# qiqiqicheng/news-recommendation-tc

Measured on AMD Instinct MI355X. Metric: recalled pairs/sec (YouTubeDNN top-30) + DIN scored pairs/sec, 1/2/4/8 MI355X, higher is better.
Workload: dtype fp16

## Files before the change

news-recommendation-tc_amd/csrc/ip_topk.hip:

```cpp
#include "nrk_common.h"

#include <float.h>
#include <math.h>
#include <stdlib.h>

#include <algorithm>
#include <type_traits>
#include <utility>

namespace nrk {

typedef float f32x16 __attribute__((ext_vector_type(16)));
typedef _Float16 f16x8 __attribute__((ext_vector_type(8)));
typedef unsigned u32x4 __attribute__((ext_vector_type(4)));
typedef float f32x4 __attribute__((ext_vector_type(4)));

constexpr int IP_KFAST = 128;
constexpr int IP_KMAX = 2048;
#ifndef NRK_SCAN_TILE
#define NRK_SCAN_TILE 8192
#endif
constexpr int SCAN_TILE = NRK_SCAN_TILE;
#ifndef NRK_SCAN_TB128
#define NRK_SCAN_TB128 4
#endif
__host__ __device__ constexpr int scan_tb(int dp) {
    return dp == 128 ? NRK_SCAN_TB128 : (64 * dp >= SCAN_TILE ? 1 : SCAN_TILE / (64 * dp));
}
constexpr int IP_SEL = 512;
constexpr int IP_BQ = 288;
constexpr int IP_KRING = 256;
constexpr size_t CATALOG_HDR = 256;

__host__ __device__ static inline int pad_dim(int d) {
    return d <= 16 ? 16 : d <= 32 ? 32 : d <= 64 ? 64 : d <= 128 ? 128 : 256;
}
__host__ __device__ static inline int64_t n_blocks_of(int64_t n_items) { return (n_items + 31) / 32; }

struct CatalogHdr {
    float max_norm;
    float max_abs;
    float scale;
    int32_t dim;
    int32_t dp;
    float max_dnorm;
};

__device__ __forceinline__ float pow2_scale(float maxabs) {
    if (!(maxabs > 0.0f)) return 1.0f;
    int e;
    (void)frexpf(maxabs, &e);
    return ldexpf(1.0f, 14 - e);
}

static inline size_t catalog_body_bytes(int64_t n_items, int dp) {
    return (size_t)n_blocks_of(n_items) * 64u * (size_t)dp;
}
__host__ __device__ static inline bool catalog_has_hb(int dp) { return dp <= 64; }
__host__ __device__ static inline size_t catalog_hb_offset(int64_t n_items, int dp) {
// ... 1185 lines not shown
        if (user < n_users) {
            acnt[(size_t)user * 2 + h] = (int)cnt[g];
            if (h == 0) reinterpret_cast<float*>(uinfo + user)[0] = live[g] ? lb : -INFINITY;
        }
    }
    if constexpr (MT <= 32) {
        if (bnd != nullptr) {
#pragma unroll
            for (int g = 0; g < UGB; ++g)
                list_bound_out<MT>(t[g], live[g], h, ubase + (gb + g) * 32 + q, n_users, jk, bnd, bnd_m, uinfo);
        }
    }
}

__device__ __forceinline__ uint32_t fkey(float f) {
    const uint32_t b = __float_as_uint(f);
    return (b >> 31) ? ~b : (b | 0x80000000u);
}
__device__ __forceinline__ float fkey_inv(uint32_t k) {
    return __uint_as_float((k >> 31) ? (k & 0x7FFFFFFFu) : ~k);
}

template <int E>
__device__ __forceinline__ void lds_ranks(const uint32_t* __restrict__ row, int c, const uint32_t (&mine)[E],
                                          int pos, int (&rank)[E]) {
#pragma unroll
    for (int e = 0; e < E; ++e) rank[e] = 0;
    for (int j0 = 0; j0 < c; j0 += 4) {
        const uint4 q = *reinterpret_cast<const uint4*>(row + j0);
        const uint32_t qq[4] = {q.x, q.y, q.z, q.w};
#pragma unroll
        for (int t = 0; t < 4; ++t) {
#pragma unroll
            for (int e = 0; e < E; ++e)
                rank[e] += (qq[t] > mine[e] || (qq[t] == mine[e] && j0 + t < e * WAVE + pos)) ? 1 : 0;
        }
    }
}

__device__ __forceinline__ uint32_t wave_sort_desc_u32(uint32_t x, int lane) {
    static_for<6>([&](auto klc) {
        constexpr int kl = decltype(klc)::value + 1, k = 1 << kl;
        static_for<kl>([&](auto jc) {
            constexpr int j = 1 << (kl - 1 - decltype(jc)::value);
            const uint32_t y = lane_xor<j>(x);
            const bool up = (lane & k) == 0;
            const bool lower = (lane & j) == 0;
            x = (lower == up) ? max(x, y) : min(x, y);
        });
    });
    return x;
}

__device__ __forceinline__ uint32_t lds_select(uint32_t* __restrict__ row, int c, int r, int lane) {
    if (c <= WAVE) {
        wave_sync_lds();
        const uint32_t srt = wave_sort_desc_u32(lane < c ? row[lane] : 0u, lane);
        return (uint32_t)__builtin_amdgcn_readlane((int)srt, r);
    }
    if (lane < 4) row[c + lane] = 0u;
    wave_sync_lds();
    uint32_t x = 0u;
    for (int b0 = 0; b0 < c; b0 += WAVE) {
        const uint32_t mine[1] = {b0 + lane < c ? row[b0 + lane] : 0u};
        int rank[1];
        lds_ranks<1>(row, c, mine, b0 + lane, rank);
        const unsigned long long b = __ballot(b0 + lane < c && rank[0] == r);
        if (b) {
            x = (uint32_t)__shfl((int)mine[0], __ffsll((long long)b) - 1, WAVE);
            break;
        }
    }
    return x;
}

#ifndef NRK_SH_WG
#define NRK_SH_WG 6
#endif
constexpr int SH_WG_PER_CU = NRK_SH_WG;
constexpr int SH_ENT = 4;

__device__ __forceinline__ void sh_load(const uint2* s0, const uint2* s1, int a0, int n, int b0, int lane,
                                        uint2 (&ent)[SH_ENT]) {
#pragma unroll
    for (int j = 0; j < SH_ENT; ++j) {
        const int e = b0 + j * WAVE + lane;
        ent[j] = e < n ? (e < a0 ? s0[e] : s1[e - a0]) : make_uint2(0u, 0u);
    }
}

__global__ __launch_bounds__(256) void ip_select_kernel(
    int64_t n_users, int k, int m2, int bandcap, const uint2* __restrict__ app,
    const int32_t* __restrict__ acnt, const float4* __restrict__ uinfo, uint2* __restrict__ cand,
    int32_t* __restrict__ cand_cnt, float2* __restrict__ ucut, int32_t* __restrict__ ovf_flag,
    int32_t* __restrict__ ovf_list, int32_t* __restrict__ ovf_count) {
    __shared__ __attribute__((aligned(16))) uint32_t sel[4][IP_SEL + 4];
    const int lane = threadIdx.x & 63, wave = threadIdx.x >> 6;
    const int64_t nw = (int64_t)gridDim.x * 4;
    const unsigned long long lt = (1ull << lane) - 1ull;
    int64_t u = (int64_t)blockIdx.x * 4 + wave;
    int2 ac_n = make_int2(0, 0);
    float4 inf_n = make_float4(0.f, 0.f, 0.f, 0.f);
    if (u < n_users) {
        ac_n = reinterpret_cast<const int2*>(acnt)[u];
        inf_n = uinfo[u];
    }
// ... 71 lines not shown
    for (int64_t u = blockIdx.x * (int64_t)blockDim.x + threadIdx.x; u < n_users;
         u += (int64_t)gridDim.x * blockDim.x) {
        cand_cnt[u] = 0;
        ovf_flag[u] = 1;
        ovf_list[u] = (int32_t)u;
    }
    if (blockIdx.x == 0 && threadIdx.x == 0) *ovf_count = (int32_t)n_users;
}

__device__ __forceinline__ double exact_dot(const float* __restrict__ a, const float* __restrict__ b,
                                            int dim) {
    double s = 0.0;
    if ((dim & 31) == 0) {
        const float4* a4 = reinterpret_cast<const float4*>(a);
        const float4* b4 = reinterpret_cast<const float4*>(b);
        for (int t0 = 0; t0 < dim / 4; t0 += 8) {
            float4 x[8], y[8];
#pragma unroll
            for (int t = 0; t < 8; ++t) {
                x[t] = a4[t0 + t];
                y[t] = b4[t0 + t];
            }
#pragma unroll
            for (int t = 0; t < 8; ++t) {
                s += (double)x[t].x * (double)y[t].x;
                s += (double)x[t].y * (double)y[t].y;
                s += (double)x[t].z * (double)y[t].z;
                s += (double)x[t].w * (double)y[t].w;
            }
        }
    } else if ((dim & 3) == 0) {
        const float4* a4 = reinterpret_cast<const float4*>(a);
        const float4* b4 = reinterpret_cast<const float4*>(b);
        for (int t = 0; t < dim / 4; ++t) {
            const float4 x = a4[t], y = b4[t];
            s += (double)x.x * (double)y.x;
            s += (double)x.y * (double)y.y;
            s += (double)x.z * (double)y.z;
            s += (double)x.w * (double)y.w;
        }
    } else {
        for (int t = 0; t < dim; ++t) s += (double)a[t] * (double)b[t];
    }
    return s + 0.0;
}

#ifndef NRK_REFINE_DIRECT
#define NRK_REFINE_DIRECT 1
#endif
constexpr bool REFINE_DIRECT = NRK_REFINE_DIRECT;
#ifndef NRK_REFINE_WPE
#define NRK_REFINE_WPE 6
#endif
template <int DS4, int SV>
__global__ __launch_bounds__(256) __attribute__((amdgpu_waves_per_eu(DS4 == 16 ? 2 : DS4 == 0 ? 4 : NRK_REFINE_WPE))) void ip_refine_kernel(
    const float* __restrict__ users, int64_t n_users, const float* __restrict__ items,
    const uint8_t* __restrict__ catalog, int64_t n_items, int dim, int k, int64_t row_offset,
    const uint2* __restrict__ cand, int bandcap, const int32_t* __restrict__ cand_cnt,
    const float2* __restrict__ ucut, const int32_t* __restrict__ ovf_flag, int32_t* __restrict__ ovf_list,
    int32_t* __restrict__ ovf_count, float* __restrict__ out_s, int32_t* __restrict__ out_r,
    double* __restrict__ out_e, int n_src = 0,
    int64_t src_users = 0, int x_cap = 0, const int32_t* __restrict__ src_cnt = nullptr) {
    constexpr int SE = SV / WAVE;
    __shared__ Cand surv[4][SV];
    __shared__ int32_t krow[4][IP_KRING];
    constexpr int RS = DS4 + 1;
    __shared__ float4 stage[DS4 > 0 ? 4 : 1][DS4 > 0 ? 32 * RS : 1];
    __shared__ uint32_t bandq[4][SV + 32 > IP_BQ ? SV + 32 : IP_BQ];
    __shared__ __attribute__((aligned(16))) float ushl[4][DS4 > 0 ? 1 : 256];
    const int lane = threadIdx.x & 63, wave = threadIdx.x >> 6;
    const int64_t u = (int64_t)blockIdx.x * 4 + wave;
    if (u >= n_users) return;
    const bool slots = n_src == 0;
    const float* uv = users + u * dim;
    const int32_t ovf_u = ovf_flag[u];
    const int nbd_slots = slots ? cand_cnt[u] : 0;
    const float2 ce = ucut[u];
    const float uv_r = uv[lane < dim ? lane : 0];
    const uint2 ent0 = slots ? cand[(size_t)u * bandcap + (lane < 32 ? lane : 0)] : make_uint2(0u, 0u);
    if (ovf_u) return;
    int src_n = 0;
    int nsrc_tot = 0;
    if (n_src > 0) {
        for (int s0 = 0; s0 < n_src; s0 += WAVE) {
            const int sl = s0 + lane;
            const int c = sl < n_src ? max(0, src_cnt[(int64_t)sl * src_users + u]) : 0;
            if (s0 == 0) src_n = c;
            nsrc_tot += (int)wave_sum_f32((float)c);
        }
    }
    if (nsrc_tot > IP_BQ) {
        if ((threadIdx.x & 63) == 0) ovf_list[atomicAdd(ovf_count, 1)] = (int32_t)u;
        return;
    }
    const float uv_l = lane < dim ? uv_r : 0.0f;
    float nz = fabsf(uv_l), uam = fabsf(uv_l);
    for (int d = lane + WAVE; d < dim; d += WAVE) {
        nz += fabsf(uv[d]);
        uam = fmaxf(uam, fabsf(uv[d]));
    }
    nz = wave_sum_f32(nz);
    if (nz == 0.0f) {
        for (int i = lane; i < k; i += WAVE) {
            const bool ok = i < n_items;
            out_s[u * k + i] = ok ? 0.0f : -FLT_MAX;
            out_r[u * k + i] = ok ? (int32_t)(i + row_offset) : -1;
            if (out_e) out_e[u * k + i] = ok ? 0.0 : -INFINITY;
// ... 19 lines not shown
        float ua = uam;
#pragma unroll
        for (int m = 32; m > 0; m >>= 1) ua = fmaxf(ua, __shfl_xor(ua, m, WAVE));
        const float su = pow2_scale(ua);
        if constexpr (DS4 > 0) {
#pragma unroll
            for (int d = lane; d < 4 * DS4; d += WAVE) ush[d] = (_Float16)(uv[d] * su);
            wave_sync_lds();
        }
        pcut = ce.x * (su * hdr->scale);
    }
    int nband = 0;
    auto take_one = [&](uint2 ent, int e, int cnt) {
        const bool kp = e < cnt && (!pre || __uint_as_float(ent.x) >= pcut);
        const unsigned long long bal = __ballot(kp);
        if (kp) bandq[wave][nband + __popcll(bal & ((1ull << lane) - 1ull))] = ent.y;
        nband += __popcll(bal);
    };
    auto take = [&](const uint2* __restrict__ src, int cnt) {
        int b0 = 0;
        if (slots) {
            take_one(ent0, lane < 32 ? lane : cnt, cnt);
            b0 = 32;
        }
        for (; b0 < cnt; b0 += WAVE) {
            const int e = b0 + lane;
            take_one(e < cnt ? src[e] : make_uint2(0u, 0u), e, cnt);
        }
    };
    if (n_src > 0) {
        const uint32_t* ids = reinterpret_cast<const uint32_t*>(cand);
        for (int s2 = 0; s2 < n_src; ++s2) {
            const int c2 = s2 < WAVE ? __shfl(src_n, s2, WAVE) : max(0, src_cnt[(int64_t)s2 * src_users + u]);
            const uint32_t* src = ids + ((size_t)s2 * src_users + u) * x_cap;
            for (int b0 = 0; b0 < c2; b0 += WAVE) {
                const int e = b0 + lane;
                if (e < c2) bandq[wave][nband + e] = src[e];
                nband += min(WAVE, c2 - b0);
            }
        }
    } else {
        take(bd, nbd);
    }
    wave_sync_lds();
    const int nitem = nband * 16;
    int cnt = 0;
    auto push = [&](bool keep, double s, int32_t row) {
        const unsigned long long bal = __ballot(keep);
        const int pos = cnt + __popcll(bal & ((1ull << lane) - 1ull));
        if (keep && pos < SV) surv[wave][pos] = Cand{s, row};
        cnt += __popcll(bal);
    };
    if constexpr (DS4 > 0) {
        uint4 pc[DSK > 0 ? 2 * DSK : 1];
        auto band_q = [&](int base) -> uint32_t {
            int idx = base + lane;
            idx = idx < nitem ? idx : nitem - 1;
            return bandq[wave][idx > 0 ? idx >> 4 : 0];
        };
        const uint8_t* hbc = catalog ? catalog + catalog_hb_offset(n_items, 4 * DS4) : nullptr;
        int64_t hoff = 0;
        auto item_row = [&](int base, uint32_t qv, int32_t& row, bool& inb) {
            const int idx = base + lane, r = idx & 15;
            const int64_t rr = (int64_t)(qv >> 1) * 32 + (r & 3) + 8 * (r >> 2) + 4 * (qv & 1);
            inb = idx < nitem && rr < n_items;
            row = inb ? (int32_t)rr : 0;
            hoff = inb ? ((int64_t)qv * 16 + r) * (8 * DS4) : 0;
        };
        auto pieces = [&](int32_t) {
            if (pre) {
                const uint8_t* bp = hbc + hoff;
#pragma unroll
                for (int st = 0; st < DSK; ++st)
#pragma unroll
                    for (int hh = 0; hh < 2; ++hh)
                        pc[2 * st + hh] = *reinterpret_cast<const uint4*>(bp + 32 * st + 16 * hh);
            }
        };
        int kc = 0, ko = 0;
        auto exact_round = [&](int m) {
            const int32_t rl = lane < m ? krow[wave][(ko + lane) & (IP_KRING - 1)] : -1;
            double sd = 0.0;
            bool keep = false;
            if constexpr (REFINE_DIRECT && DS4 <= 8) {
                if (rl >= 0) {
                    const float4* a4 = reinterpret_cast<const float4*>(uv);
                    const float4* b4 = reinterpret_cast<const float4*>(items + (int64_t)rl * dim);
                    constexpr int YH = DS4 > 4 ? DS4 / 2 : DS4;
                    double acc = 0.0;
#pragma unroll
                    for (int t0 = 0; t0 < DS4; t0 += YH) {
                        float4 y[YH];
#pragma unroll
                        for (int t = 0; t < YH; ++t) y[t] = b4[t0 + t];
#pragma unroll
                        for (int t = 0; t < YH; ++t) {
                            const float4 x = a4[t0 + t];
                            acc += (double)x.x * (double)y[t].x;
                            acc += (double)x.y * (double)y[t].y;
                            acc += (double)x.z * (double)y[t].z;
                            acc += (double)x.w * (double)y[t].w;
                        }
                    }
                    sd = acc + 0.0;
                    keep = sd >= thr;
                }
                push(keep, sd, rl);
                ko += m;
                return;
            }
#pragma unroll
            for (int hp = 0; hp < 2; ++hp) {
                float4 v[DS4 / 2];
                bool okv[DS4 / 2];
#pragma unroll
                for (int it = 0; it < DS4 / 2; ++it) {
                    const int g = it * 64 + lane, item = 32 * hp + g / DS4, part = g % DS4;
                    const int r_item = __shfl(rl, item, WAVE);
                    okv[it] = r_item >= 0;
                    v[it] = reinterpret_cast<const float4*>(items + (int64_t)(okv[it] ? r_item : 0) * dim)[part];
                }
#pragma unroll
                for (int it = 0; it < DS4 / 2; ++it) {
                    const int g = it * 64 + lane, part = g % DS4;
                    stage[wave][(g / DS4) * RS + part] = okv[it] ? v[it] : make_float4(0.f, 0.f, 0.f, 0.f);
                }
                wave_sync_lds();
                if ((lane >> 5) == hp && rl >= 0) {
                    const float4* a4 = reinterpret_cast<const float4*>(uv);
                    const float4* b4 = &stage[wave][(lane & 31) * RS];
                    double acc = 0.0;
#pragma unroll
                    for (int t = 0; t < DS4; ++t) {
                        const float4 x = a4[t], y = b4[t];
                        acc += (double)x.x * (double)y.x;
                        acc += (double)x.y * (double)y.y;
                        acc += (double)x.z * (double)y.z;
                        acc += (double)x.w * (double)y.w;
                    }
                    sd = acc + 0.0;
                    keep = sd >= thr;
                }
                wave_sync_lds();
            }
            push(keep, sd, rl);
            ko += m;
        };
        int32_t row;
        bool inb;
        item_row(0, band_q(0), row, inb);
        pieces(row);
        uint32_t q1 = band_q(WAVE < nitem ? WAVE : 0);
        for (int base = 0; base < nitem; base += WAVE) {
            bool keep = inb;
            if (pre && inb) {
                float acc = 0.0f;
#pragma unroll
                for (int st = 0; st < DSK; ++st)
#pragma unroll
                    for (int hh = 0; hh < 2; ++hh) {
                        const f16x8 hv = __builtin_bit_cast(f16x8, pc[2 * st + hh]);
                        const f16x8 uh = *reinterpret_cast<const f16x8*>(&ush[16 * st + 8 * hh]);
#pragma unroll
                        for (int e = 0; e < 8; ++e)
                            acc = fmaf((float)hv[e], (float)uh[e], acc);
                    }
                keep = acc >= pcut;
            }
            const int32_t row_cur = row;
            const int nb = base + WAVE;
            if (nb < nitem) {
                item_row(nb, q1, row, inb);
                pieces(row);
                q1 = band_q(nb + WAVE < nitem ? nb + WAVE : nb);
            }
            const unsigned long long bal = __ballot(keep);
            if (keep) krow[wave][(kc + __popcll(bal & ((1ull << lane) - 1ull))) & (IP_KRING - 1)] = row_cur;
            kc += __popcll(bal);
            wave_sync_lds();
            while (kc - ko >= WAVE) exact_round(WAVE);
        }
        while (kc > ko) exact_round(kc - ko < WAVE ? kc - ko : WAVE);
    } else {
        const int dpc = pad_dim(dim), dskc = dpc / 16;
        if (pre) {
            float ua = 0.0f;
            for (int d = 0; d < dim; ++d) ua = fmaxf(ua, fabsf(uv[d]));
            const float s2 = pow2_scale(ua);
            for (int d = lane; d < dpc; d += WAVE) ushl[wave][d] = d < dim ? (float)(_Float16)(uv[d] * s2) : 0.0f;
            wave_sync_lds();
        }
        int kc = 0, ko = 0;
        auto exact_generic = [&](int m) {
            const int32_t rl = lane < m ? krow[wave][(ko + lane) & (IP_KRING - 1)] : -1;
            double sd = 0.0;
            bool keep = false;
            if (rl >= 0) {
                sd = exact_dot(uv, items + (int64_t)rl * dim, dim);
                keep = sd >= thr;
            }
            push(keep, sd, rl);
            ko += m;
        };
        for (int base = 0; base < nitem; base += WAVE) {
            const int idx = base + lane;
            bool keep = false;
            int32_t row = 0;
            if (idx < nitem) {
                const int bb = idx >> 4, r = idx & 15;
                const uint32_t qv = bandq[wave][bb];
                const int64_t rr = (int64_t)(qv >> 1) * 32 + (r & 3) + 8 * (r >> 2) + 4 * (qv & 1);
                if (rr < n_items) row = (int32_t)rr;
                keep = rr < n_items;
                if (keep && pre) {
                    const uint8_t* bp = catalog + (size_t)(rr >> 5) * (64 * dpc);
                    const int il = (int)(rr & 31);
                    float acc = 0.0f;
                    for (int st = 0; st < dskc; ++st) {
                        const f16x8 h0 = __builtin_bit_cast(f16x8, *reinterpret_cast<const uint4*>(bp + st * 1024 + il * 16));
                        const f16x8 h1 =
                            __builtin_bit_cast(f16x8, *reinterpret_cast<const uint4*>(bp + st * 1024 + (il + 32) * 16));
                        const float* us = &ushl[wave][16 * st];
#pragma unroll
                        for (int e = 0; e < 8; ++e) acc = fmaf((float)h0[e], us[e], acc);
#pragma unroll
                        for (int e = 0; e < 8; ++e) acc = fmaf((float)h1[e], us[8 + e], acc);
                    }
                    keep = acc >= pcut;
                }
            }
            const unsigned long long bal = __ballot(keep);
            if (keep) krow[wave][(kc + __popcll(bal & ((1ull << lane) - 1ull))) & (IP_KRING - 1)] = row;
            kc += __popcll(bal);
            wave_sync_lds();
            while (kc - ko >= WAVE) exact_generic(WAVE);
        }
        while (kc > ko) exact_generic(kc - ko < WAVE ? kc - ko : WAVE);
    }
    if (cnt > SV) {
        if (lane == 0) ovf_list[atomicAdd(ovf_count, 1)] = (int32_t)u;
        return;
    }
    wave_sync_lds();
    auto emit = [&](const Cand* x, int ne) {
        for (int e = 0; e < ne; ++e) {
            const int idx = e * 64 + lane;
            if (idx < k) {
                const bool ok = x[e].row != INT32_MAX;
                out_s[u * k + idx] = ok ? (float)x[e].s : -FLT_MAX;
                out_r[u * k + idx] = ok ? (int32_t)(x[e].row + row_offset) : -1;
                if (out_e) out_e[u * k + idx] = ok ? x[e].s : -INFINITY;
            }
        }
    };
    if (SE > 1 && cnt <= WAVE && k <= WAVE) {
        Cand x1[1];
        if (lane < cnt) x1[0] = surv[wave][lane];
        else { x1[0].s = -INFINITY; x1[0].row = INT32_MAX; }
        wave_bitonic_sort<1>(x1);
        emit(x1, 1);
        return;
    }
    Cand x[SE];
#pragma unroll
    for (int e = 0; e < SE; ++e) {
        const int idx = e * 64 + lane;
        if (idx < cnt) x[e] = surv[wave][idx];
        else { x[e].s = -INFINITY; x[e].row = INT32_MAX; }
    }
    wave_bitonic_sort<SE>(x);
    emit(x, SE);
}

__device__ __forceinline__ uint64_t okey(double s) {
    const uint64_t b = (uint64_t)__double_as_longlong(s);
    return (b >> 63) ? ~b : (b | 0x8000000000000000ull);
}

constexpr int FB_GRID = 256;

__global__ __launch_bounds__(256) void ip_exact_kernel(
    const float* __restrict__ users, const float* __restrict__ items, int64_t n_items, int dim, int k, int ns,
    int64_t row_offset, const int32_t* __restrict__ ovf_list, const int32_t* __restrict__ ovf_count,
    float* __restrict__ out_s, int32_t* __restrict__ out_r, double* __restrict__ out_e,
    uint32_t* __restrict__ scratch, int32_t* __restrict__ slow_list, int32_t* __restrict__ slow_count) {
    extern __shared__ __attribute__((aligned(16))) uint8_t dyn[];
    Cand* sel = reinterpret_cast<Cand*>(dyn);
    __shared__ unsigned int hist[2048];
    __shared__ unsigned int part[256];
    __shared__ int s_bin, s_krem, s_eq, sel_n;
    const int tid = threadIdx.x, lane = tid & 63;
    const int cnt = *ovf_count;
    const int kk = (int)(n_items < k ? n_items : k);
    uint32_t* key = scratch + (size_t)blockIdx.x * n_items;
    for (int qi = blockIdx.x; qi < cnt; qi += gridDim.x) {
        const int64_t u = ovf_list[qi];
        const float* uv = users + u * dim;
        for (int64_t r = tid; r < n_items; r += 256) key[r] = fkey((float)exact_dot(uv, items + r * dim, dim));
        __syncthreads();
        uint32_t prefix = 0, mask = 0;
        int krem = kk;
        for (int p = 0; p < 3; ++p) {
            const int wbits = p < 2 ? 11 : 10, sh = p == 0 ? 21 : (p == 1 ? 10 : 0);
            const uint32_t nbm = (1u << wbits) - 1u;
            for (int i = tid; i < 2048; i += 256) hist[i] = 0u;
            __syncthreads();
            for (int64_t r0 = 0; r0 < n_items; r0 += 256) {
                const int64_t r = r0 + tid;
// ... 611 lines not shown
    launch_scan_v<DP, NW, NSL, UG, MT, WPE>(users, n_users, cat, n_items, dim, k, w, s);
}

template <int DP>
static void launch_scan_k(const float* users, int n_users, const uint8_t* cat, int n_items, int dim, int k,
                          const IpWs& w, hipStream_t s) {
    const int mt = (k + 1) / 2;
    if (mt <= 16) launch_scan<DP, 16>(users, n_users, cat, n_items, dim, k, w, s);
    else if (mt <= 32) launch_scan<DP, 32>(users, n_users, cat, n_items, dim, k, w, s);
    else launch_scan<DP, 64>(users, n_users, cat, n_items, dim, k, w, s);
}

static void scan_dispatch(const float* users, int nu, const uint8_t* cat, int ni, int dim, int k, const IpWs& w,
                          hipStream_t s) {
    switch (pad_dim(dim)) {
        case 16: launch_scan_k<16>(users, nu, cat, ni, dim, k, w, s); break;
        case 32: launch_scan_k<32>(users, nu, cat, ni, dim, k, w, s); break;
        case 64: launch_scan_k<64>(users, nu, cat, ni, dim, k, w, s); break;
        case 128: launch_scan_k<128>(users, nu, cat, ni, dim, k, w, s); break;
        default: launch_scan_k<256>(users, nu, cat, ni, dim, k, w, s); break;
    }
}

static int ip_range(IpWs& w, int64_t n_items, int dim, int64_t blk_lo, int64_t blk_hi) {
    const int tb = scan_tb(pad_dim(dim));
    NRK_REQUIRE(blk_lo >= 0 && blk_lo <= blk_hi && blk_hi <= n_blocks_of(n_items), "block range out of bounds");
    NRK_REQUIRE(blk_lo == blk_hi || (blk_lo % tb == 0 && (blk_hi % tb == 0 || blk_hi == n_blocks_of(n_items))),
                "block range must start (and end, unless at the catalog end) on a 8-KB tile");
    w.blk_lo = (int)blk_lo;
    w.blk_hi = (int)blk_hi;
    return NRK_OK;
}

static inline bool shard_listbound(int k) { return (k + 1) / 2 <= 32; }

static int sh_grid(int64_t n_users) {
    return (int)std::max<int64_t>(1, std::min<int64_t>((n_users + 3) / 4, (int64_t)n_cus() * SH_WG_PER_CU));
}

__global__ void ip_empty_range_kernel(int64_t n_users, int32_t* __restrict__ acnt, float4* __restrict__ uinfo) {
    for (int64_t u = blockIdx.x * (int64_t)blockDim.x + threadIdx.x; u < n_users;
         u += (int64_t)gridDim.x * blockDim.x) {
        acnt[2 * u] = 0;
        acnt[2 * u + 1] = 0;
        uinfo[u] = make_float4(-INFINITY, 0.0f, 0.0f, 0.0f);
    }
}

static void launch_exact(const float* users, int64_t n_users, const float* items, int64_t n_items, int dim, int k,
                         int64_t row_offset, const IpWs& w, float* out_s, int32_t* out_r, double* out_e,
                         hipStream_t s) {
    const int ns = next_pow2(std::max(k, 64));
    const size_t lds = (size_t)ns * sizeof(Cand);
    (void)hipFuncSetAttribute((const void*)ip_exact_kernel, hipFuncAttributeMaxDynamicSharedMemorySize, (int)lds);
    (void)hipFuncSetAttribute((const void*)ip_fallback_kernel, hipFuncAttributeMaxDynamicSharedMemorySize, (int)lds);
    const int grid = (int)std::min<int64_t>(n_users, FB_GRID);
    ip_exact_kernel<<<grid, 256, lds, s>>>(users, items, n_items, dim, k, ns, row_offset, w.ovf_list, w.ovf_count,
                                           out_s, out_r, out_e, w.fbk, w.slow_list, w.ovf_count + 1);
    ip_fallback_kernel<<<grid, 256, lds, s>>>(users, items, n_items, dim, k, ns, row_offset, w.slow_list,
                                              w.ovf_count + 1, out_s, out_r, out_e);
}

}

using namespace nrk;

extern "C" {

#if NRK_SCAN_STAMP
int nrk_dev_scan_stamps(unsigned long long* out) {
    return hipMemcpyFromSymbol(out, HIP_SYMBOL(scan_stamps), sizeof(scan_stamps)) == hipSuccess ? 0 : -1;
}
#endif

int nrk_ip_topk_tile_blocks(int dim) {
    if (dim <= 0 || dim > 256) return 0;
    return scan_tb(pad_dim(dim));
}

size_t nrk_ip_catalog_bytes(int64_t n_items, int dim) {
    if (n_items < 0 || dim <= 0 || dim > 256) return 0;
    const int dp = pad_dim(dim);
    return catalog_body_bytes(n_items, dp) + CATALOG_HDR + (catalog_has_hb(dp) ? catalog_body_bytes(n_items, dp) : 0);
}

int nrk_ip_catalog_build(const float* items, int64_t n_items, int dim, void* catalog,
                         nrk_stream_t stream) {
    clear_error();
    NRK_REQUIRE(items != nullptr || n_items == 0, "items is null");
    NRK_REQUIRE(catalog != nullptr, "catalog is null");
    NRK_REQUIRE(n_items >= 0 && n_items < INT32_MAX, "n_items out of range");
    NRK_REQUIRE(dim > 0 && dim <= 256, "dim must be in [1, 256]");
    const int dp = pad_dim(dim);
    hipStream_t s = as_stream(stream);
    const size_t body = catalog_body_bytes(n_items, dp);
    CatalogHdr* hdr = reinterpret_cast<CatalogHdr*>(reinterpret_cast<uint8_t*>(catalog) + body);
    if (hipMemsetAsync(hdr, 0, CATALOG_HDR, s) != hipSuccess) {
        set_error("nrk_ip_catalog_build: hipMemsetAsync failed");
        return NRK_EHIP;
    }
    const int64_t total = n_blocks_of(n_items) * (dp / 16) * 64;
    if (total > 0) {
        const int g2 = (int)std::min<int64_t>((n_items + 15) / 16, 2048);
        catalog_norm_kernel<<<g2, 256, 0, s>>>(items, n_items, dim, hdr);
    }
    catalog_hdr_kernel<<<1, 1, 0, s>>>(hdr, dim, dp);
    if (total > 0) {
        const int g2 = (int)std::min<int64_t>((n_items + 15) / 16, 2048);
// ... 54 lines not shown
        }
        if (n_items == 0) {
            (void)hipMemsetAsync(w.cnt, 0, (size_t)n_users * sizeof(int32_t), s);
            (void)hipMemsetAsync(w.ovf_flag, 0, (size_t)n_users * sizeof(int32_t), s);
            (void)hipMemsetAsync(w.ucut, 0xFF, (size_t)n_users * sizeof(float2), s);
        } else if (k > IP_KFAST) {
            const int grid = (int)std::min<int64_t>((n_users + 255) / 256, 4096);
            ip_all_exact_kernel<<<grid, 256, 0, s>>>(n_users, w.cnt, w.ovf_flag, w.ovf_list, w.ovf_count);
        } else {
            ip_select_kernel<<<sh_grid(n_users), 256, 0, s>>>(n_users, k, w.m2, w.bandcap, w.app, w.acnt, w.uinfo,
                                                              w.cand, w.cnt, w.ucut, w.ovf_flag, w.ovf_list,
                                                              w.ovf_count);
        }
    }
    NRK_CHECK_LAUNCH();
    return NRK_OK;
}

int nrk_ip_topk_scan(const float* users, int64_t n_users, const void* catalog, int64_t n_items, int dim, int k,
                     void* workspace, size_t workspace_bytes, nrk_stream_t stream) {
    clear_error();
    return screen_phases(users, n_users, catalog, n_items, dim, k, 0, n_blocks_of(n_items), workspace,
                         workspace_bytes, stream, 1);
}

int nrk_ip_topk_select(const float* users, int64_t n_users, const void* catalog, int64_t n_items, int dim, int k,
                       void* workspace, size_t workspace_bytes, nrk_stream_t stream) {
    clear_error();
    return screen_phases(users, n_users, catalog, n_items, dim, k, 0, n_blocks_of(n_items), workspace,
                         workspace_bytes, stream, 2);
}

int nrk_ip_topk_screen(const float* users, int64_t n_users, const void* catalog, int64_t n_items,
                       int dim, int k, void* workspace, size_t workspace_bytes,
                       nrk_stream_t stream) {
    clear_error();
    return screen_phases(users, n_users, catalog, n_items, dim, k, 0, n_blocks_of(n_items), workspace,
                         workspace_bytes, stream, 3);
}

int nrk_ip_topk_finish(const float* users, int64_t n_users, const float* items,
                       const void* catalog, int64_t n_items,
                       int dim, int k, int64_t row_offset, float* out_scores, int32_t* out_rows,
                       double* out_exact, void* workspace, size_t workspace_bytes,
                       nrk_stream_t stream) {
    clear_error();
    int rc = ip_check(users, n_users, items, items, n_items, dim, k, workspace, workspace_bytes);
    if (rc != NRK_OK || n_users == 0) return rc;
    NRK_REQUIRE(out_scores && out_rows, "null output");
    const IpWs w = ip_ws_layout(workspace, n_users, n_items, k, dim);
    hipStream_t s = as_stream(stream);
    const int g2 = (int)((n_users + 3) / 4);
    const uint8_t* cat = reinterpret_cast<const uint8_t*>(catalog);
#define NRK_REFINE(DS4, SV)                                                                                  \
    ip_refine_kernel<DS4, SV><<<g2, 256, 0, s>>>(users, n_users, items, cat, n_items, dim, k, row_offset,   \
                                                 w.cand, w.bandcap, w.cnt, w.ucut, w.ovf_flag, w.ovf_list,   \
                                                 w.ovf_count, out_scores, out_rows, out_exact)
#define NRK_REFINE_SV(DS4)                          \
    do {                                            \
        if (k <= 64) NRK_REFINE(DS4, 128);          \
        else NRK_REFINE(DS4, 256);                  \
    } while (0)
    if (k <= IP_KFAST || n_items == 0) {
        if (dim == 32) NRK_REFINE_SV(8);
        else if (dim == 16) NRK_REFINE_SV(4);
        else if (dim == 64) NRK_REFINE_SV(16);
        else NRK_REFINE_SV(0);
    }
#undef NRK_REFINE_SV
#undef NRK_REFINE
    if (n_items > 0) launch_exact(users, n_users, items, n_items, dim, k, row_offset, w, out_scores, out_rows, out_exact, s);
    NRK_CHECK_LAUNCH();
    return NRK_OK;
}

int nrk_ip_topk(const float* users, int64_t n_users, const float* items, const void* catalog,
                int64_t n_items, int dim, int k, int64_t row_offset, float* out_scores,
                int32_t* out_rows, double* out_exact, void* workspace, size_t workspace_bytes,
                nrk_stream_t stream) {
    int rc = nrk_ip_topk_screen(users, n_users, catalog, n_items, dim, k, workspace,
                                workspace_bytes, stream);
    if (rc != NRK_OK) return rc;
    return nrk_ip_topk_finish(users, n_users, items, catalog, n_items, dim, k, row_offset, out_scores,
                              out_rows, out_exact, workspace, workspace_bytes, stream);
}

int nrk_ip_topk_bound(const float* users, int64_t n_users, const void* catalog, int64_t n_items, int dim,
                      int k, int m, float* out_bound, void* workspace, size_t workspace_bytes,
                      nrk_stream_t stream) {
    clear_error();
    int rc = ip_check(users, n_users, (const float*)catalog, catalog, n_items, dim, k, workspace,
                      workspace_bytes);
    if (rc != NRK_OK) return rc;
    if (k > IP_KFAST) NRK_UNSUPPORTED("the screen bound needs k <= 128");
    NRK_REQUIRE(m >= 1 && m <= 256, "m must be in [1, 256]");
    if (n_users == 0) return NRK_OK;
    NRK_REQUIRE(out_bound != nullptr, "null pointer");
    const IpWs w = ip_ws_layout(workspace, n_users, n_items, k, dim);
    hipStream_t s = as_stream(stream);
    if (n_items == 0) {
        (void)hipMemsetAsync(w.cnt, 0, (size_t)n_users * sizeof(int32_t), s);
    }
    const CatalogHdr* hdr = reinterpret_cast<const CatalogHdr*>(
        reinterpret_cast<const uint8_t*>(catalog) + catalog_body_bytes(n_items, pad_dim(dim)));
    const int grid = (int)((n_users + 3) / 4);
    const int need = std::max(w.bandcap, m);
#define NRK_BOUND(E, NS)                                                                                    \
    ip_bound_kernel<E><<<grid, 256, (E) ? 0 : 4 * (NS) * sizeof(Cand), s>>>(users, n_users, dim, hdr, w.cand, \
                                                                           w.bandcap, w.cnt, w.ucut, m, NS,  \
                                                                           out_bound)
    if (need <= 64) NRK_BOUND(1, 64);
    else if (need <= 128) NRK_BOUND(2, 128);
    else if (need <= 256) NRK_BOUND(4, 256);
    else NRK_BOUND(0, next_pow2(need));
// ... 59 lines not shown
        scan_dispatch(users, (int)n_users, reinterpret_cast<const uint8_t*>(catalog), (int)n_items, dim, k, w, s);
    }
    if (!lbnd)
        ip_shard_bound_kernel<<<sh_grid(n_users), 256, 0, s>>>(n_users, w.m2, w.app, w.acnt, w.uinfo, m, out_bound,
                                                               w.ovf_flag, w.bandcap, w.cand, w.cnt);
    NRK_CHECK_LAUNCH();
    return NRK_OK;
}

int nrk_ip_topk_shard_band(int64_t n_users, int64_t n_items, int dim, int k, const float* bounds, int n_lists,
                           int m, int x_cap, void* workspace, size_t workspace_bytes, void* out_ent,
                           int32_t* out_cnt, nrk_stream_t stream) {
    clear_error();
    NRK_REQUIRE(x_cap >= 1 && x_cap <= IP_BQ, "x_cap must be in [1, 288]");
    NRK_REQUIRE(n_users >= 0 && n_users < (1ll << 30) && n_items >= 0 && dim > 0 && dim <= 256, "bad sizes");
    NRK_REQUIRE(k >= 1 && k <= IP_KFAST, "k must be in [1, 128]");
    NRK_REQUIRE(bounds == nullptr || (n_lists >= 1 && m >= 1 && n_lists * m <= 512),
                "need 1 <= n_lists * m <= 512");
    if (n_users == 0) return NRK_OK;
    NRK_REQUIRE(workspace && out_ent && out_cnt, "null pointer");
    NRK_REQUIRE(workspace_bytes >= ip_ws_layout(nullptr, n_users, n_items, k, dim).bytes, "workspace too small");
    const IpWs w = ip_ws_layout(workspace, n_users, n_items, k, dim);
    ip_shard_band_kernel<<<sh_grid(n_users), 256, 0, as_stream(stream)>>>(
        n_users, k, w.m2, w.app, w.acnt, w.uinfo, bounds, bounds ? n_lists : 0, bounds ? m : 1, w.bandcap,
        shard_listbound(k) ? nullptr : w.ovf_flag, shard_listbound(k) ? nullptr : w.cand,
        shard_listbound(k) ? nullptr : w.cnt, w.ucut, reinterpret_cast<uint32_t*>(out_ent), out_cnt, x_cap);
    NRK_CHECK_LAUNCH();
    return NRK_OK;
}

int nrk_ip_topk_refine_x(const float* users, int64_t n_users, const float* items, const void* catalog,
                         int64_t n_items, int dim, int k, int64_t row_offset, const void* band, int n_src,
                         int64_t src_users, int x_cap, const int32_t* src_cnt, const float* ucut,
                         const int32_t* ovf_in, float* out_scores, int32_t* out_rows, double* out_exact,
                         void* workspace, size_t workspace_bytes, nrk_stream_t stream) {
    clear_error();
    int rc = ip_check(users, n_users, items, items, n_items, dim, k, workspace, workspace_bytes);
    if (rc != NRK_OK || n_users == 0) return rc;
    NRK_REQUIRE(out_scores && out_rows && band && src_cnt && ucut, "null pointer");
    NRK_REQUIRE(n_src >= 1 && x_cap >= 1 && src_users >= n_users, "need n_src >= 1, x_cap >= 1, src_users >= n_users");
    if (k > IP_KFAST) NRK_UNSUPPORTED("the band refine needs k <= 128 (larger k: exact path, ovf_in = 1)");
    const IpWs w = ip_ws_layout(workspace, n_users, n_items, k, dim);
    hipStream_t s = as_stream(stream);
    if (hipMemsetAsync(w.ovf_count, 0, 256, s) != hipSuccess) {
        set_error("nrk_ip_topk_refine_x: hipMemsetAsync failed");
        return NRK_EHIP;
    }
    ip_ovf_collect_kernel<<<(int)std::min<int64_t>((n_users + 255) / 256, 4096), 256, 0, s>>>(
        n_users, ovf_in, w.ovf_flag, w.ovf_list, w.ovf_count);
    const int g2 = (int)((n_users + 3) / 4);
    const uint8_t* cat = reinterpret_cast<const uint8_t*>(catalog);
    const uint2* bd = reinterpret_cast<const uint2*>(band);
    const float2* uc = reinterpret_cast<const float2*>(ucut);
#define NRK_REFINE(DS4, SV)                                                                                   \
    ip_refine_kernel<DS4, SV><<<g2, 256, 0, s>>>(users, n_users, items, cat, n_items, dim, k, row_offset, bd, 0, \
                                                 nullptr, uc, w.ovf_flag, w.ovf_list, w.ovf_count, out_scores,   \
                                                 out_rows, out_exact, n_src, src_users, x_cap, src_cnt)
#define NRK_REFINE_SV(DS4)                 \
    do {                                   \
        if (k <= 64) NRK_REFINE(DS4, 128); \
        else NRK_REFINE(DS4, 256);         \
    } while (0)
    if (dim == 32) NRK_REFINE_SV(8);
    else if (dim == 16) NRK_REFINE_SV(4);
    else if (dim == 64) NRK_REFINE_SV(16);
    else NRK_REFINE_SV(0);
#undef NRK_REFINE_SV
#undef NRK_REFINE
    if (n_items > 0) launch_exact(users, n_users, items, n_items, dim, k, row_offset, w, out_scores, out_rows, out_exact, s);
    NRK_CHECK_LAUNCH();
    return NRK_OK;
}

int nrk_topk_merge(const double* in_exact, const int32_t* in_rows, int n_lists, int64_t list_stride,
                   int64_t n_users, int k_in, int k_out, float* out_scores, int32_t* out_rows,
                   double* out_exact, nrk_stream_t stream) {
    clear_error();
    NRK_REQUIRE(n_lists >= 1 && k_in >= 1 && k_out >= 1 && n_users >= 0, "bad sizes");
    NRK_REQUIRE(list_stride >= n_users * (int64_t)k_in, "list_stride too small");
    const int tot = n_lists * k_in;
    if (tot > 1024) NRK_UNSUPPORTED("n_lists * k_in > 1024");
    NRK_REQUIRE(k_out <= tot, "k_out > n_lists * k_in");
    if (n_users == 0) return NRK_OK;
    NRK_REQUIRE(in_exact && in_rows && out_scores && out_rows, "null pointer");
    hipStream_t s = as_stream(stream);
    const int grid = (int)((n_users + 3) / 4);
#define NRK_MERGE(E, NS)                                                                                    \
    topk_merge_kernel<E><<<grid, 256, (E) ? 0 : 4 * (NS) * sizeof(Cand), s>>>(in_exact, in_rows, n_lists,      \
                                                                              list_stride, n_users, k_in, k_out, \
                                                                              NS, out_scores, out_rows, out_exact)
    if (tot <= 64) NRK_MERGE(1, 64);
    else if (tot <= 128) NRK_MERGE(2, 128);
    else if (tot <= 256) NRK_MERGE(4, 256);
    else NRK_MERGE(0, next_pow2(tot));
#undef NRK_MERGE
    NRK_CHECK_LAUNCH();
    return NRK_OK;
}

}
```

Baseline: 1.214 billion.

## Split half-precision prefilter across lanes, add 64-bit key sort fast path

```diff
diff --git a/news-recommendation-tc_amd/csrc/ip_topk.hip b/news-recommendation-tc_amd/csrc/ip_topk.hip
--- a/news-recommendation-tc_amd/csrc/ip_topk.hip
+++ b/news-recommendation-tc_amd/csrc/ip_topk.hip
@@ -5,6 +5,7 @@
 #include <stdlib.h>
 
 #include <algorithm>
+#include <atomic>
 #include <type_traits>
 #include <utility>
 
@@ -1296,6 +1297,26 @@
     return x;
 }
 
+constexpr uint64_t lanes_bit_clear(int b) {
+    uint64_t m = 0;
+    for (int l = 0; l < 64; ++l) m |= (uint64_t)((l & b) == 0) << l;
+    return m;
+}
+
+__device__ __forceinline__ uint64_t wave_sort_desc_u64(uint64_t x) {
+    static_for<6>([&](auto klc) {
+        constexpr int kl = decltype(klc)::value + 1, k = 1 << kl;
+        static_for<kl>([&](auto jc) {
+            constexpr int j = 1 << (kl - 1 - decltype(jc)::value);
+            constexpr uint64_t KEEP_MIN = lanes_bit_clear(j) ^ lanes_bit_clear(k);
+            const uint64_t y = ((uint64_t)lane_xor<j>((uint32_t)(x >> 32)) << 32) | (uint64_t)lane_xor<j>((uint32_t)x);
+            const bool keep_x = __builtin_amdgcn_inverse_ballot_w64(__builtin_amdgcn_ballot_w64(x > y) ^ KEEP_MIN);
+            x = keep_x ? x : y;
+        });
+    });
+    return x;
+}
+
 __device__ __forceinline__ uint32_t lds_select(uint32_t* __restrict__ row, int c, int r, int lane) {
     if (c <= WAVE) {
         wave_sync_lds();
@@ -1473,7 +1494,13 @@
 #ifndef NRK_REFINE_WPE
 #define NRK_REFINE_WPE 6
 #endif
-template <int DS4, int SV>
+#ifndef NRK_REFINE_LANES
+#define NRK_REFINE_LANES 1
+#endif
+#ifndef NRK_REFINE_KEY64
+#define NRK_REFINE_KEY64 1
+#endif
+template <int DS4, int SV, bool FK>
 __global__ __launch_bounds__(256) __attribute__((amdgpu_waves_per_eu(DS4 == 16 ? 2 : DS4 == 0 ? 4 : NRK_REFINE_WPE))) void ip_refine_kernel(
     const float* __restrict__ users, int64_t n_users, const float* __restrict__ items,
     const uint8_t* __restrict__ catalog, int64_t n_items, int dim, int k, int64_t row_offset,
@@ -1599,34 +1626,19 @@
         cnt += __popcll(bal);
     };
     if constexpr (DS4 > 0) {
-        uint4 pc[DSK > 0 ? 2 * DSK : 1];
-        auto band_q = [&](int base) -> uint32_t {
-            int idx = base + lane;
-            idx = idx < nitem ? idx : nitem - 1;
-            return bandq[wave][idx > 0 ? idx >> 4 : 0];
-        };
+        constexpr bool LANES = NRK_REFINE_LANES && (DS4 == 4 || DS4 == 8);
         const uint8_t* hbc = catalog ? catalog + catalog_hb_offset(n_items, 4 * DS4) : nullptr;
-        int64_t hoff = 0;
-        auto item_row = [&](int base, uint32_t qv, int32_t& row, bool& inb) {
-            const int idx = base + lane, r = idx & 15;
-            const int64_t rr = (int64_t)(qv >> 1) * 32 + (r & 3) + 8 * (r >> 2) + 4 * (qv & 1);
-            inb = idx < nitem && rr < n_items;
-            row = inb ? (int32_t)rr : 0;
-            hoff = inb ? ((int64_t)qv * 16 + r) * (8 * DS4) : 0;
-        };
-        auto pieces = [&](int32_t) {
-            if (pre) {
-                const uint8_t* bp = hbc + hoff;
-#pragma unroll
-                for (int st = 0; st < DSK; ++st)
-#pragma unroll
-                    for (int hh = 0; hh < 2; ++hh)
-                        pc[2 * st + hh] = *reinterpret_cast<const uint4*>(bp + 32 * st + 16 * hh);
-            }
-        };
         int kc = 0, ko = 0;
         auto exact_round = [&](int m) {
-            const int32_t rl = lane < m ? krow[wave][(ko + lane) & (IP_KRING - 1)] : -1;
+            int32_t rl = lane < m ? krow[wave][(ko + lane) & (IP_KRING - 1)] : -1;
+            if constexpr (LANES) {
+                if (rl >= 0) {
+                    const uint32_t qv = bandq[wave][rl >> 4];
+                    const int r = rl & 15;
+                    const int64_t rr = (int64_t)(qv >> 1) * 32 + (r & 3) + 8 * (r >> 2) + 4 * (qv & 1);
+                    rl = rr < n_items ? (int32_t)rr : -1;
+                }
+            }
             double sd = 0.0;
             bool keep = false;
             if constexpr (REFINE_DIRECT && DS4 <= 8) {
@@ -1693,39 +1705,131 @@
             push(keep, sd, rl);
             ko += m;
         };
-        int32_t row;
-        bool inb;
-        item_row(0, band_q(0), row, inb);
-        pieces(row);
-        uint32_t q1 = band_q(WAVE < nitem ? WAVE : 0);
-        for (int base = 0; base < nitem; base += WAVE) {
-            bool keep = inb;
-            if (pre && inb) {
-                float acc = 0.0f;
-#pragma unroll
-                for (int st = 0; st < DSK; ++st)
-#pragma unroll
-                    for (int hh = 0; hh < 2; ++hh) {
-                        const f16x8 hv = __builtin_bit_cast(f16x8, pc[2 * st + hh]);
-                        const f16x8 uh = *reinterpret_cast<const f16x8*>(&ush[16 * st + 8 * hh]);
-#pragma unroll
-                        for (int e = 0; e < 8; ++e)
-                            acc = fmaf((float)hv[e], (float)uh[e], acc);
+        if constexpr (LANES) {
+            constexpr int LPI = DS4 / 2, HS = 4 / LPI, WL = 16 * LPI;
+            constexpr int LGL = LPI == 4 ? 2 : 1;
+            const int sub = lane & (LPI - 1), itl = lane >> LGL;
+            const uint32_t woff = (uint32_t)(lane & (WL - 1)) * 16u;
+            const uint32_t nhb1 = (uint32_t)(2 * ((n_items + 31) >> 5)) - 1u;
+            const int ngrp = (nband + 3) >> 2;
+            auto group_q = [&](int g) -> uint32_t {
+                return min(bandq[wave][min(4 * g + (lane & 3), nband - 1)], nhb1);
+            };
+            auto loads = [&](uint32_t qg, uint4(&p)[LPI]) {
+#pragma unroll
+                for (int t = 0; t < LPI; ++t) {
+                    uint32_t q = (uint32_t)__builtin_amdgcn_readlane((int)qg, HS * t);
+                    if constexpr (HS == 2) {
+                        const uint32_t q1 = (uint32_t)__builtin_amdgcn_readlane((int)qg, 2 * t + 1);
+                        q = lane < 32 ? q : q1;
                     }
-                keep = acc >= pcut;
-            }
-            const int32_t row_cur = row;
-            const int nb = base + WAVE;
-            if (nb < nitem) {
-                item_row(nb, q1, row, inb);
-                pieces(row);
-                q1 = band_q(nb + WAVE < nitem ? nb + WAVE : nb);
-            }
-            const unsigned long long bal = __ballot(keep);
-            if (keep) krow[wave][(kc + __popcll(bal & ((1ull << lane) - 1ull))) & (IP_KRING - 1)] = row_cur;
-            kc += __popcll(bal);
-            wave_sync_lds();
-            while (kc - ko >= WAVE) exact_round(WAVE);
+                    p[t] = *reinterpret_cast<const uint4*>(hbc + (q * (uint32_t)(128 * DS4) + woff));
+                }
+            };
+            auto score = [&](const uint4(&p)[LPI]) -> float {
+                const f16x8 uh = *reinterpret_cast<const f16x8*>(&ush[8 * sub]);
+                float a[LPI];
+#pragma unroll
+                for (int t = 0; t < LPI; ++t) {
+                    const f16x8 hv = __builtin_bit_cast(f16x8, p[t]);
+                    float acc = 0.0f;
+#pragma unroll
+                    for (int e = 0; e < 8; ++e) acc = fmaf((float)hv[e], (float)uh[e], acc);
+                    acc += __int_as_float(__builtin_amdgcn_update_dpp(0, __float_as_int(acc), 0xB1, 0xF, 0xF, true));
+                    if constexpr (LPI == 4)
+                        acc += __int_as_float(__builtin_amdgcn_update_dpp(0, __float_as_int(acc), 0x4E, 0xF, 0xF, true));
+                    a[t] = acc;
+                }
+                float r = (sub & 1) ? a[1] : a[0];
+                if constexpr (LPI == 4) {
+                    const float r2 = (sub & 1) ? a[3] : a[2];
+                    r = (sub & 2) ? r2 : r;
+                }
+                return r;
+            };
+            uint4 pc[LPI] = {};
+            uint32_t qn = 0;
+            if (pre && ngrp > 0) {
+                loads(group_q(0), pc);
+                qn = group_q(ngrp > 1 ? 1 : 0);
+            }
+            for (int g = 0; g < ngrp; ++g) {
+                const int hb = 4 * g + HS * sub + (itl >> 4);
+                bool keep = hb < nband;
+                if (pre) {
+                    const float sc = score(pc);
+                    keep = keep && sc >= pcut;
+                    if (g + 1 < ngrp) {
+                        loads(qn, pc);
+                        qn = group_q(g + 2 < ngrp ? g + 2 : g + 1);
+                    }
+                }
+                const unsigned long long bal = __ballot(keep);
+                if (keep)
+                    krow[wave][(kc + __popcll(bal & ((1ull << lane) - 1ull))) & (IP_KRING - 1)] = hb * 16 + (itl & 15);
+                kc += __popcll(bal);
+                wave_sync_lds();
+                while (kc - ko >= WAVE) exact_round(WAVE);
+            }
+        } else {
+            uint4 pc[DSK > 0 ? 2 * DSK : 1];
+            auto band_q = [&](int base) -> uint32_t {
+                int idx = base + lane;
+                idx = idx < nitem ? idx : nitem - 1;
+                return bandq[wave][idx > 0 ? idx >> 4 : 0];
+            };
+            int64_t hoff = 0;
+            auto item_row = [&](int base, uint32_t qv, int32_t& row, bool& inb) {
+                const int idx = base + lane, r = idx & 15;
+                const int64_t rr = (int64_t)(qv >> 1) * 32 + (r & 3) + 8 * (r >> 2) + 4 * (qv & 1);
+                inb = idx < nitem && rr < n_items;
+                row = inb ? (int32_t)rr : 0;
+                hoff = inb ? ((int64_t)qv * 16 + r) * (8 * DS4) : 0;
+            };
+            auto pieces = [&](int32_t) {
+                if (pre) {
+                    const uint8_t* bp = hbc + hoff;
+#pragma unroll
+                    for (int st = 0; st < DSK; ++st)
+#pragma unroll
+                        for (int hh = 0; hh < 2; ++hh)
+                            pc[2 * st + hh] = *reinterpret_cast<const uint4*>(bp + 32 * st + 16 * hh);
+                }
+            };
+            int32_t row;
+            bool inb;
+            item_row(0, band_q(0), row, inb);
+            pieces(row);
+            uint32_t q1 = band_q(WAVE < nitem ? WAVE : 0);
+            for (int base = 0; base < nitem; base += WAVE) {
+                bool keep = inb;
+                if (pre && inb) {
+                    float acc = 0.0f;
+#pragma unroll
+                    for (int st = 0; st < DSK; ++st)
+#pragma unroll
+                        for (int hh = 0; hh < 2; ++hh) {
+                            const f16x8 hv = __builtin_bit_cast(f16x8, pc[2 * st + hh]);
+                            const f16x8 uh = *reinterpret_cast<const f16x8*>(&ush[16 * st + 8 * hh]);
+#pragma unroll
+                            for (int e = 0; e < 8; ++e)
+                                acc = fmaf((float)hv[e], (float)uh[e], acc);
+                        }
+                    keep = acc >= pcut;
+                }
+                const int32_t row_cur = row;
+                const int nb = base + WAVE;
+                if (nb < nitem) {
+                    item_row(nb, q1, row, inb);
+                    pieces(row);
+                    q1 = band_q(nb + WAVE < nitem ? nb + WAVE : nb);
+                }
+                const unsigned long long bal = __ballot(keep);
+                if (keep) krow[wave][(kc + __popcll(bal & ((1ull << lane) - 1ull))) & (IP_KRING - 1)] = row_cur;
+                kc += __popcll(bal);
+                wave_sync_lds();
+                while (kc - ko >= WAVE) exact_round(WAVE);
+            }
         }
         while (kc > ko) exact_round(kc - ko < WAVE ? kc - ko : WAVE);
     } else {
@@ -1801,6 +1905,24 @@
         }
     };
     if (SE > 1 && cnt <= WAVE && k <= WAVE) {
+        if constexpr (FK && NRK_REFINE_KEY64) {
+            uint64_t key = 0;
+            if (lane < cnt) {
+                const Cand c = surv[wave][lane];
+                key = ((uint64_t)fkey((float)c.s) << 32) | (uint32_t)~c.row;
+            }
+            key = wave_sort_desc_u64(key);
+            const uint32_t hi = (uint32_t)(key >> 32);
+            const uint32_t hi_next = (uint32_t)__shfl_down((int)hi, 1, WAVE);
+            if (!__ballot(lane < k && lane + 1 < cnt && hi == hi_next)) {
+                if (lane < k) {
+                    const bool ok = lane < cnt;
+                    out_s[u * k + lane] = ok ? fkey_inv(hi) : -FLT_MAX;
+                    out_r[u * k + lane] = ok ? (int32_t)((int32_t)~(uint32_t)key + row_offset) : -1;
+                }
+                return;
+            }
+        }
         Cand x1[1];
         if (lane < cnt) x1[0] = surv[wave][lane];
         else { x1[0].s = -INFINITY; x1[0].row = INT32_MAX; }
@@ -2518,8 +2640,16 @@
                          hipStream_t s) {
     const int ns = next_pow2(std::max(k, 64));
     const size_t lds = (size_t)ns * sizeof(Cand);
-    (void)hipFuncSetAttribute((const void*)ip_exact_kernel, hipFuncAttributeMaxDynamicSharedMemorySize, (int)lds);
-    (void)hipFuncSetAttribute((const void*)ip_fallback_kernel, hipFuncAttributeMaxDynamicSharedMemorySize, (int)lds);
+    static std::atomic<uint64_t> attr_done{0};
+    int dev = 0;
+    (void)hipGetDevice(&dev);
+    const uint64_t dbit = 1ull << (dev & 63);
+    if (dev >= 64 || !(attr_done.load(std::memory_order_acquire) & dbit)) {
+        const int lds_max = next_pow2(IP_KMAX) * (int)sizeof(Cand);
+        (void)hipFuncSetAttribute((const void*)ip_exact_kernel, hipFuncAttributeMaxDynamicSharedMemorySize, lds_max);
+        (void)hipFuncSetAttribute((const void*)ip_fallback_kernel, hipFuncAttributeMaxDynamicSharedMemorySize, lds_max);
+        attr_done.fetch_or(dbit, std::memory_order_release);
+    }
     const int grid = (int)std::min<int64_t>(n_users, FB_GRID);
     ip_exact_kernel<<<grid, 256, lds, s>>>(users, items, n_items, dim, k, ns, row_offset, w.ovf_list, w.ovf_count,
                                            out_s, out_r, out_e, w.fbk, w.slow_list, w.ovf_count + 1);
@@ -2680,14 +2810,15 @@
     hipStream_t s = as_stream(stream);
     const int g2 = (int)((n_users + 3) / 4);
     const uint8_t* cat = reinterpret_cast<const uint8_t*>(catalog);
-#define NRK_REFINE(DS4, SV)                                                                                  \
-    ip_refine_kernel<DS4, SV><<<g2, 256, 0, s>>>(users, n_users, items, cat, n_items, dim, k, row_offset,   \
-                                                 w.cand, w.bandcap, w.cnt, w.ucut, w.ovf_flag, w.ovf_list,   \
-                                                 w.ovf_count, out_scores, out_rows, out_exact)
-#define NRK_REFINE_SV(DS4)                          \
-    do {                                            \
-        if (k <= 64) NRK_REFINE(DS4, 128);          \
-        else NRK_REFINE(DS4, 256);                  \
+#define NRK_REFINE(DS4, SV, FK)                                                                                \
+    ip_refine_kernel<DS4, SV, FK><<<g2, 256, 0, s>>>(users, n_users, items, cat, n_items, dim, k, row_offset, \
+                                                     w.cand, w.bandcap, w.cnt, w.ucut, w.ovf_flag, w.ovf_list, \
+                                                     w.ovf_count, out_scores, out_rows, out_exact)
+#define NRK_REFINE_SV(DS4)                                  \
+    do {                                                    \
+        if (k > 64) NRK_REFINE(DS4, 256, false);            \
+        else if (out_exact) NRK_REFINE(DS4, 128, false);    \
+        else NRK_REFINE(DS4, 128, true);                    \
     } while (0)
     if (k <= IP_KFAST || n_items == 0) {
         if (dim == 32) NRK_REFINE_SV(8);
@@ -2853,14 +2984,15 @@
     const uint8_t* cat = reinterpret_cast<const uint8_t*>(catalog);
     const uint2* bd = reinterpret_cast<const uint2*>(band);
     const float2* uc = reinterpret_cast<const float2*>(ucut);
-#define NRK_REFINE(DS4, SV)                                                                                   \
-    ip_refine_kernel<DS4, SV><<<g2, 256, 0, s>>>(users, n_users, items, cat, n_items, dim, k, row_offset, bd, 0, \
-                                                 nullptr, uc, w.ovf_flag, w.ovf_list, w.ovf_count, out_scores,   \
-                                                 out_rows, out_exact, n_src, src_users, x_cap, src_cnt)
-#define NRK_REFINE_SV(DS4)                 \
-    do {                                   \
-        if (k <= 64) NRK_REFINE(DS4, 128); \
-        else NRK_REFINE(DS4, 256);         \
+#define NRK_REFINE(DS4, SV, FK)                                                                                      \
+    ip_refine_kernel<DS4, SV, FK><<<g2, 256, 0, s>>>(users, n_users, items, cat, n_items, dim, k, row_offset, bd, 0, \
+                                                     nullptr, uc, w.ovf_flag, w.ovf_list, w.ovf_count, out_scores,   \
+                                                     out_rows, out_exact, n_src, src_users, x_cap, src_cnt)
+#define NRK_REFINE_SV(DS4)                                  \
+    do {                                                    \
+        if (k > 64) NRK_REFINE(DS4, 256, false);            \
+        else if (out_exact) NRK_REFINE(DS4, 128, false);    \
+        else NRK_REFINE(DS4, 128, true);                    \
     } while (0)
     if (dim == 32) NRK_REFINE_SV(8);
     else if (dim == 16) NRK_REFINE_SV(4);
```

Result: faster. 1.250 billion, median of 6 (+3.0%).
